# snuspl/parallax

Hardware: NVIDIA H100
Metric: lm1b_words_per_sec (higher is better)
Workload: dtype bf16

## Files before the change

### parallax_b200/ops/csrc/kernels/lstm_persistent.cu

```cuda
#include <cooperative_groups.h>
#include <mutex>

#include "wgmma.cuh"
#include "lstm_cell.cuh"

namespace cg = cooperative_groups;

namespace lstm_fwd {
using namespace tc;

constexpr int UNITS = 32;
constexpr int ROWS = 64;
constexpr int GN = 2 * UNITS;
constexpr int PN = 64;
constexpr int PK = 128;
constexpr int NTHREADS = 512;
constexpr int CELL_U = 4;
constexpr int GATE_LD = 4 * UNITS + 8;
constexpr int MAX_KB = 8;

struct Args {
  const __nv_bfloat16* xw;
  const __nv_bfloat16* Wh;
  const __nv_bfloat16* WP;
  __nv_bfloat16* act;
  float* c_all;
  __nv_bfloat16* m_all;
  __nv_bfloat16* h_all;
  float* ws;
  int T, S, P;
  float forget_bias;
};

__host__ __device__ constexpr int cmax(int a, int b) { return a > b ? a : b; }
__host__ __device__ constexpr int x_bytes(int P) {
  return cmax(cmax((P / BK) * ROWS * 128, (PK / BK) * BM * 128), ROWS * GATE_LD * 4);
}
__host__ __device__ constexpr int smem_bytes(int P) {
  return 2 * (P / BK) * GN * 128 + (PK / BK) * PN * 128 + x_bytes(P) + (MAX_KB + PK / BK) * 8 + 1024;
}
static_assert(smem_bytes(MAX_KB * BK) <= 232448, "P = 512 must fit one CTA's shared memory");

template <int N, typename Col>
__device__ __forceinline__ void load_transposed(uint8_t* dst, const __nv_bfloat16* src, size_t ld,
                                                int K, Col col) {
  const int nblk = (N / 8) * (K / 8);
  for (int b = threadIdx.x; b < nblk; b += blockDim.x) {
    const int n0 = (b % (N / 8)) * 8, k0 = (b / (N / 8)) * 8;
    uint4 v[8];
#pragma unroll
    for (int i = 0; i < 8; ++i)
      v[i] = __ldg(reinterpret_cast<const uint4*>(src + (size_t)(k0 + i) * ld + col(n0)));
    const uint32_t* w = reinterpret_cast<const uint32_t*>(v);
    uint8_t* blk = dst + (k0 / BK) * N * 128;
    const int c = (k0 % BK) / 8;
#pragma unroll
    for (int j = 0; j < 8; ++j) {
      const uint32_t sel = (j & 1) ? 0x7632u : 0x5410u;
      uint4 o;
      o.x = __byte_perm(w[0 * 4 + j / 2], w[1 * 4 + j / 2], sel);
      o.y = __byte_perm(w[2 * 4 + j / 2], w[3 * 4 + j / 2], sel);
      o.z = __byte_perm(w[4 * 4 + j / 2], w[5 * 4 + j / 2], sel);
      o.w = __byte_perm(w[6 * 4 + j / 2], w[7 * 4 + j / 2], sel);
      const int n = n0 + j;
      *reinterpret_cast<uint4*>(blk + n * 128 + ((c ^ (n & 7)) << 4)) = o;
    }
  }
}

__device__ __forceinline__ float2 bf16x2_to_float2(uint32_t w) {
  return make_float2(__uint_as_float(w << 16), __uint_as_float(w & 0xffff0000u));
}
__device__ __forceinline__ uint32_t float2_to_bf16x2(float a, float b) {
  __nv_bfloat162 h = __floats2bfloat162_rn(a, b);
  return *reinterpret_cast<uint32_t*>(&h);
}
__device__ __forceinline__ float round_bf16(float x) {
  return __bfloat162float(__float2bfloat16_rn(x));
}

__device__ __forceinline__ void product(float* acc, uint32_t a0, uint32_t a_stride, uint32_t b0,
                                        uint64_t* bar, int nkb, uint32_t parity) {
  for (int kb = 0; kb < nkb; ++kb) {
    mbar_wait(&bar[kb], parity);
    const uint64_t adesc = make_smem_desc(a0 + kb * a_stride);
    const uint64_t bdesc = make_smem_desc(b0 + kb * 64 * 128);
    wgmma_fence();
#pragma unroll
    for (int k = 0; k < BK / WG_K; ++k)
      wgmma_bf16<64>(acc, adesc + (uint64_t)(k * 2), bdesc + (uint64_t)(k * 2),
                     (kb | k) != 0 ? 1u : 0u);
    wgmma_commit();
  }
  wgmma_wait<0>();
}

__global__ void __launch_bounds__(NTHREADS, 1)
px_lstm_fwd_persistent_kernel(const __grid_constant__ CUtensorMap tmap_h,
                              const __grid_constant__ CUtensorMap tmap_m, Args a) {
  extern __shared__ __align__(1024) uint8_t smem_raw[];
  uint8_t* smem = reinterpret_cast<uint8_t*>(((uintptr_t)smem_raw + 1023) & ~(uintptr_t)1023);
  const int S = a.S, P = a.P, KB = P / BK;
  const size_t G4 = 4 * (size_t)S;
  uint8_t* sWh = smem;
  uint8_t* sWP = sWh + 2 * KB * GN * 128;
  uint8_t* sX = sWP + (PK / BK) * PN * 128;
  uint64_t* hbar = reinterpret_cast<uint64_t*>(sX + x_bytes(P));
  uint64_t* mbar = hbar + MAX_KB;

  const int row0 = (blockIdx.x & 1) * ROWS, u0 = (blockIdx.x >> 1) * UNITS;
  const int ntn = P / PN;
  const bool proj = (int)blockIdx.x < ntn * (S / PK);
  const int pn0 = (blockIdx.x % ntn) * PN, pk = blockIdx.x / ntn;

  if (threadIdx.x == 0) {
    asm volatile("prefetch.tensormap [%0];" ::"l"(&tmap_h) : "memory");
    asm volatile("prefetch.tensormap [%0];" ::"l"(&tmap_m) : "memory");
    for (int kb = 0; kb < KB; ++kb) mbar_init(&hbar[kb], 1);
    for (int kb = 0; kb < PK / BK; ++kb) mbar_init(&mbar[kb], 1);
    asm volatile("fence.mbarrier_init.release.cluster;" ::: "memory");
  }
  for (int w = 0; w < 2; ++w)
    load_transposed<GN>(sWh + w * KB * GN * 128, a.Wh, G4, P,
                        [=](int n) { return (n / 16) * S + u0 + 16 * w + n % 16; });
  if (proj)
    load_transposed<PN>(sWP, a.WP + (size_t)pk * PK * P, P, PK, [=](int n) { return pn0 + n; });
  asm volatile("fence.proxy.async.shared::cta;" ::: "memory");
  __syncthreads();

  const int wg = threadIdx.x >> 7, lane = threadIdx.x & 31, warp = (threadIdx.x >> 5) & 3;
  const int q2 = (lane & 3) * 2;
  const int r = warp * 16 + (lane >> 2);
  const int rb = wg * 64 + r;
  const int crow = threadIdx.x / (UNITS / CELL_U), cu = (threadIdx.x % (UNITS / CELL_U)) * CELL_U;
  const size_t cs_off = (size_t)(row0 + crow) * S + u0 + cu;
  const size_t cg_off = (size_t)(row0 + crow) * G4 + u0 + cu;
  float c[CELL_U];
  {
    const float4 v = *reinterpret_cast<const float4*>(a.c_all + cs_off);
    c[0] = v.x; c[1] = v.y; c[2] = v.z; c[3] = v.w;
  }
  float* sG = reinterpret_cast<float*>(sX);
  const uint32_t sX_u = smem_u32(sX), sWh_u = smem_u32(sWh) + (wg & 1) * KB * GN * 128;
  const uint32_t sWP_u = smem_u32(sWP);
  cg::grid_group grid = cg::this_grid();
  const int KS = S / PK;
  float acc[32];

  for (int t = 0; t < a.T; ++t) {
    const uint32_t parity = t & 1;
    if (threadIdx.x == 0) {
      asm volatile("fence.proxy.async.global;" ::: "memory");
      for (int kb = 0; kb < KB; ++kb) {
        mbar_expect_tx(&hbar[kb], ROWS * BK * 2);
        tma_load_2d(sX + kb * ROWS * 128, &tmap_h, &hbar[kb], kb * BK, t * BM + row0);
      }
    }
    uint2 xv[4];
    const __nv_bfloat16* xr = a.xw + (size_t)t * BM * G4 + cg_off;
#pragma unroll
    for (int g = 0; g < 4; ++g) xv[g] = __ldg(reinterpret_cast<const uint2*>(xr + (size_t)g * S));
    if (wg < 2) {
      product(acc, sX_u, ROWS * 128, sWh_u, hbar, KB, parity);
      consumer_sync();
#pragma unroll
      for (int h = 0; h < 2; ++h)
#pragma unroll
        for (int j = 0; j < GN / 8; ++j)
          *reinterpret_cast<float2*>(sG + (r + 8 * h) * GATE_LD + (j >> 1) * UNITS + wg * 16 +
                                     (j & 1) * 8 + q2) =
              make_float2(acc[j * 4 + 2 * h], acc[j * 4 + 2 * h + 1]);
    }
    __syncthreads();

    float av[4][CELL_U], mv[CELL_U];
#pragma unroll
    for (int g = 0; g < 4; ++g) {
      const float4 v = *reinterpret_cast<const float4*>(sG + crow * GATE_LD + g * UNITS + cu);
      const float2 lo = bf16x2_to_float2(xv[g].x), hi = bf16x2_to_float2(xv[g].y);
      av[g][0] = round_bf16(v.x + lo.x);
      av[g][1] = round_bf16(v.y + lo.y);
      av[g][2] = round_bf16(v.z + hi.x);
      av[g][3] = round_bf16(v.w + hi.y);
    }
    asm volatile("fence.proxy.async.shared::cta;" ::: "memory");
#pragma unroll
    for (int e = 0; e < CELL_U; ++e) {
      float ae[4];
      c[e] = lstm_cell_fwd_elem(av[0][e], av[1][e], av[2][e], av[3][e], c[e], a.forget_bias, ae,
                                &mv[e]);
#pragma unroll
      for (int g = 0; g < 4; ++g) av[g][e] = ae[g];
    }
    __nv_bfloat16* act = a.act + (size_t)t * BM * G4 + cg_off;
#pragma unroll
    for (int g = 0; g < 4; ++g)
      *reinterpret_cast<uint2*>(act + (size_t)g * S) =
          make_uint2(float2_to_bf16x2(av[g][0], av[g][1]), float2_to_bf16x2(av[g][2], av[g][3]));
    *reinterpret_cast<float4*>(a.c_all + (size_t)(t + 1) * BM * S + cs_off) =
        make_float4(c[0], c[1], c[2], c[3]);
    *reinterpret_cast<uint2*>(a.m_all + (size_t)t * BM * S + cs_off) =
        make_uint2(float2_to_bf16x2(mv[0], mv[1]), float2_to_bf16x2(mv[2], mv[3]));
    grid.sync();

    if (proj && wg < 2) {
      if (threadIdx.x == 0) {
        asm volatile("fence.proxy.async.global;" ::: "memory");
        for (int kb = 0; kb < PK / BK; ++kb) {
          mbar_expect_tx(&mbar[kb], BM * BK * 2);
          tma_load_2d(sX + kb * BM * 128, &tmap_m, &mbar[kb], pk * PK + kb * BK, t * BM);
        }
      }
      product(acc, sX_u + wg * 64 * 128, BM * 128, sWP_u, mbar, PK / BK, parity);
      float* slot = a.ws + (size_t)pk * BM * P;
#pragma unroll
      for (int h = 0; h < 2; ++h)
#pragma unroll
        for (int j = 0; j < PN / 8; ++j)
          *reinterpret_cast<float2*>(slot + (size_t)(rb + 8 * h) * P + pn0 + j * 8 + q2) =
              make_float2(acc[j * 4 + 2 * h], acc[j * 4 + 2 * h + 1]);
    }
    grid.sync();

    __nv_bfloat16* hn = a.h_all + (size_t)(t + 1) * BM * P;
    const int npairs = BM * P / 2;
    for (int i = blockIdx.x * blockDim.x + threadIdx.x; i < npairs; i += gridDim.x * blockDim.x) {
      float2 s = __ldcg(reinterpret_cast<const float2*>(a.ws) + i);
#pragma unroll 8
      for (int k = 1; k < KS; ++k) {
        const float2 v = __ldcg(reinterpret_cast<const float2*>(a.ws + (size_t)k * BM * P) + i);
        s.x += v.x;
        s.y += v.y;
      }
      reinterpret_cast<uint32_t*>(hn)[i] = float2_to_bf16x2(s.x, s.y);
    }
    if (t + 1 < a.T) grid.sync();
  }
}

}

extern "C" {

int px_lstm_fwd_persistent_grid(int B, int S, int P) {
  using namespace lstm_fwd;
  if (B != BM || S <= 0 || S % PK || P <= 0 || P % PN || P > MAX_KB * BK) return 0;
  static std::mutex mu;
  static int cap[16][MAX_KB + 1];
  int dev = 0;
  if (cudaGetDevice(&dev) != cudaSuccess || dev < 0 || dev >= 16) return 0;
  std::lock_guard<std::mutex> lock(mu);
  int& n = cap[dev][P / PN];
  if (n == 0) {
    int coop = 0, sms = 0, per_sm = 0;
    cudaDeviceGetAttribute(&coop, cudaDevAttrCooperativeLaunch, dev);
    cudaDeviceGetAttribute(&sms, cudaDevAttrMultiProcessorCount, dev);
    const int smem = smem_bytes(P);
    if (cudaFuncSetAttribute(px_lstm_fwd_persistent_kernel,
                             cudaFuncAttributeMaxDynamicSharedMemorySize,
                             smem_bytes(MAX_KB * BK)) != cudaSuccess ||
        cudaOccupancyMaxActiveBlocksPerMultiprocessor(&per_sm, px_lstm_fwd_persistent_kernel,
                                                      NTHREADS, smem) != cudaSuccess)
      per_sm = 0;
    n = (coop && per_sm > 0) ? per_sm * sms : -1;
    cudaGetLastError();
  }
  const int grid = 2 * (S / UNITS);
  return n >= grid ? grid : 0;
}

int px_lstm_fwd_persistent(const void* xw, const void* Wh, const void* WP, void* act, float* c_all,
                           void* m_all, void* h_all, float* ws, int T, int B, int S, int P,
                           float forget_bias, cudaStream_t stream) {
  using namespace lstm_fwd;
  const int grid = px_lstm_fwd_persistent_grid(B, S, P);
  if (grid <= 0 || T < 1) return -1;
  for (const void* q : {xw, Wh, WP, (const void*)act, (const void*)c_all, (const void*)m_all,
                        (const void*)h_all, (const void*)ws})
    if ((uintptr_t)q % 16) return -1;
  CUtensorMap th, tm;
  int rc = make_tmap(&th, h_all, (uint64_t)(T + 1) * B, P, ROWS);
  if (rc) return rc;
  rc = make_tmap(&tm, m_all, (uint64_t)T * B, S, BM);
  if (rc) return rc;
  Args a;
  a.xw = (const __nv_bfloat16*)xw; a.Wh = (const __nv_bfloat16*)Wh;
  a.WP = (const __nv_bfloat16*)WP; a.act = (__nv_bfloat16*)act; a.c_all = c_all;
  a.m_all = (__nv_bfloat16*)m_all; a.h_all = (__nv_bfloat16*)h_all; a.ws = ws;
  a.T = T; a.S = S; a.P = P; a.forget_bias = forget_bias;
  cudaLaunchConfig_t cfg = {};
  cfg.gridDim = dim3(grid);
  cfg.blockDim = dim3(NTHREADS);
  cfg.dynamicSmemBytes = smem_bytes(P);
  cfg.stream = stream;
  cudaLaunchAttribute at[1];
  at[0].id = cudaLaunchAttributeCooperative;
  at[0].val.cooperative = 1;
  cfg.attrs = at;
  cfg.numAttrs = 1;
  const cudaError_t e = cudaLaunchKernelEx(&cfg, px_lstm_fwd_persistent_kernel, th, tm, a);
  return e == cudaSuccess ? (int)cudaGetLastError() : (int)e;
}

}
```

### parallax_b200/ops/fused.py

```python
import ctypes

import torch

from . import lib as _lib, check as _check, register_signatures

_vp, _i, _f = ctypes.c_void_p, ctypes.c_int, ctypes.c_float
register_signatures({
    "px_lstm_cell_fwd": (_i, [_vp, _vp, _vp, _vp, _vp, _i, _i, _f, _i, _vp]),
    "px_lstm_cell_bwd": (_i, [_vp, _vp, _vp, _vp, _vp, _vp, _i, _i, _i, _vp]),
    "px_lstm_dm_cell_bwd": (_i, [_vp] * 7 + [_i, _i, _i, _i, _vp]),
    "px_lstm_fwd_persistent_grid": (_i, [_i, _i, _i]),
    "px_lstm_fwd_persistent": (_i, [_vp] * 8 + [_i, _i, _i, _i, _f, _vp]),
    "px_sampled_softmax": (_i, [_vp, _vp, _vp, _vp, _vp, _vp, _vp, _vp, _i, _i, _i, _vp]),
    "px_sampled_softmax_dot": (_i, [_vp, _vp, _vp, _i, _vp, _vp, _vp, _vp, _vp, _vp, _i, _i, _i,
                                    _vp]),
    "px_ssm_bwd": (_i, [_vp, _vp, _vp, _vp, _i, _vp, _vp, _f, _vp, _vp, _vp, _i, _vp, _i, _i, _i,
                        _vp]),
})
_DT = {torch.float32: 0, torch.bfloat16: 1}


def _p(t):
    return _vp(t.data_ptr())


def _stream():
    return _vp(torch.cuda.current_stream().cuda_stream)


def _count(n=1):
    from ..parallel import nvops
    nvops.launches["n"] += n


def _acc(t):
    return t if t.dtype == torch.float64 else t.float()


BWD_BN = 16


def _fused_bwd_ok(dt, Bsz, S, P, W_P):
    return (dt == torch.bfloat16 and Bsz % 128 == 0 and S % BWD_BN == 0 and P % 64 == 0 and
            W_P.is_contiguous() and W_P.data_ptr() % 16 == 0)


_persistent_grid = {}


def _fwd_persistent_ok(dt, Bsz, S, P, Wh, W_P):
    if not (dt == torch.bfloat16 and Wh.is_contiguous() and W_P.is_contiguous() and
            Wh.data_ptr() % 16 == 0 and W_P.data_ptr() % 16 == 0):
        return False
    key = (torch.cuda.current_device(), Bsz, S, P)
    if key not in _persistent_grid:
        _persistent_grid[key] = _lib().px_lstm_fwd_persistent_grid(Bsz, S, P)
    return _persistent_grid[key] > 0


def lstm_layer_reference(x, Wx, Wh, bias, W_P, c0, h0, forget_bias=1.0):
    T, Bsz, E = x.shape
    S = W_P.shape[0]
    xw = torch.addmm(bias, x.reshape(T * Bsz, E), Wx).view(T, Bsz, 4 * S)
    c, h, outs = _acc(c0), h0, []
    for t in range(T):
        gates = _acc(torch.addmm(xw[t], h, Wh))
        i, j, f, o = gates.split(S, dim=1)
        c = torch.sigmoid(f + forget_bias) * c + torch.sigmoid(i) * torch.tanh(j)
        m = (torch.sigmoid(o) * torch.tanh(c)).to(x.dtype)
        h = m @ W_P
        outs.append(h)
    return torch.stack(outs), c, h


class _LSTMLayerFn(torch.autograd.Function):

    @staticmethod
    def forward(ctx, x, W, Wh, bias, W_P, c0, h0, forget_bias):
        L = _lib()
        T, Bsz, E = x.shape
        S, P = W_P.shape
        dt = x.dtype
        dev = x.device
        x = x.contiguous()
        stacked = Wh is None
        ctx.stacked = stacked
        ctx.param_refs = (W, bias, W_P)
        if stacked:
            Wx, Wh = W.detach()[:E], W.detach()[E:]
        else:
            Wx = W
        if any(ctx.needs_input_grad) and not _fused_bwd_ok(dt, Bsz, S, P, W_P):
            from . import sinks
            cur = torch.cuda.current_stream(dev)
            ws = sinks.side_stream(dev)
            ws.wait_stream(cur)
            with torch.cuda.stream(ws):
                ctx.WPT = W_P.detach().t().contiguous()
                ctx.WPT_ev = torch.cuda.Event()
                ctx.WPT_ev.record(ws)
            ctx.WPT.record_stream(cur)
        xw = torch.addmm(bias, x.view(T * Bsz, E), Wx).view(T, Bsz, 4 * S)
        act = torch.empty(T, Bsz, 4 * S, dtype=dt, device=dev)
        c_all = torch.empty(T + 1, Bsz, S, dtype=torch.float32, device=dev)
        m_all = torch.empty(T, Bsz, S, dtype=dt, device=dev)
        h_all = torch.empty(T + 1, Bsz, P, dtype=dt, device=dev)
        c_all[0].copy_(c0)
        h_all[0].copy_(h0)
        st = _stream()
        if _fwd_persistent_ok(dt, Bsz, S, P, Wh, W_P):
            ws = torch.empty(S // 128, Bsz, P, dtype=torch.float32, device=dev)
            _check(L.px_lstm_fwd_persistent(_p(xw), _p(Wh), _p(W_P), _p(act), _p(c_all),
                                            _p(m_all), _p(h_all), _p(ws), T, Bsz, S, P,
                                            float(forget_bias), st), "lstm_fwd_persistent")
            _count(1)
        else:
            for t in range(T):
                gpre = xw[t].addmm_(h_all[t], Wh)
                _check(L.px_lstm_cell_fwd(_p(gpre), _p(c_all[t]), _p(act[t]),
                                          _p(c_all[t + 1]), _p(m_all[t]), Bsz, S,
                                          float(forget_bias), _DT[dt], st), "lstm_cell_fwd")
                torch.mm(m_all[t], W_P, out=h_all[t + 1])
            _count(T)
        ctx.save_for_backward(x, Wx, Wh, W_P, act, c_all, m_all, h_all)
        ctx.dims = (T, Bsz, E, S, P)
        return h_all[1:], c_all[T].clone(), h_all[T].clone()

    @staticmethod
    def backward(ctx, dH, dcT, dhT):
        from . import sinks
        L = _lib()
        x, Wx, Wh, W_P, act, c_all, m_all, h_all = ctx.saved_tensors
        T, Bsz, E, S, P = ctx.dims
        stacked = ctx.stacked
        W_ref, bias_ref, WP_ref = ctx.param_refs
        dt, dev = x.dtype, x.device
        dH = dH.contiguous()
        dgates = torch.empty(T, Bsz, 4 * S, dtype=dt, device=dev)
        dh_tot = torch.empty(T, Bsz, P, dtype=dt, device=dev)
        dc = torch.zeros(Bsz, S, dtype=torch.float32, device=dev) if dcT is None \
            else dcT.float().clone()
        dh_rec = None if dhT is None else dhT.to(dt)
        fused = _fused_bwd_ok(dt, Bsz, S, P, W_P)
        dm = None if fused else torch.empty(Bsz, S, dtype=dt, device=dev)
        cur = torch.cuda.current_stream(dev)
        if not fused:
            cur.wait_event(ctx.WPT_ev)
            WPT = ctx.WPT
        from . import gemm as _gemm
        use_tc = (dt == torch.bfloat16 and Bsz % 128 == 0 and P % 64 == 0 and
                  (4 * S) % 1024 == 0 and Wh.is_contiguous())
        WhT = None if use_tc else Wh.t().contiguous()
        st = _stream()

        def sink_of(ref, shape):
            s_ = sinks.get(ref)
            if s_ is not None and s_.dtype == dt and tuple(s_.shape) == tuple(shape):
                return s_, True
            return torch.empty(shape, dtype=dt, device=dev), False
        if stacked:
            dW, w_sunk = sink_of(W_ref, (E + P, 4 * S))
            dWx_o, dWh_o = dW[:E], dW[E:]
        else:
            dWx_o, w_sunk = sink_of(W_ref, (E, 4 * S))
            dWh_o = torch.empty(P, 4 * S, dtype=dt, device=dev)
        dbias_o, b_sunk = sink_of(bias_ref, (4 * S,))
        dWP_o, p_sunk = sink_of(WP_ref, (S, P))
        ws = sinks.side_stream(dev)
        ws2 = sinks.side_stream(dev, 1)
        if dh_rec is None:
            dh_tot[T - 1].copy_(dH[T - 1])
        else:
            torch.add(dH[T - 1], dh_rec, out=dh_tot[T - 1])
        for t in range(T - 1, -1, -1):
            if fused:
                _check(L.px_lstm_dm_cell_bwd(_p(dh_tot[t]), _p(W_P), _p(dc), _p(act[t]),
                                             _p(c_all[t]), _p(c_all[t + 1]), _p(dgates[t]), Bsz,
                                             S, P, BWD_BN, st), "lstm_dm_cell_bwd")
            else:
                torch.mm(dh_tot[t], WPT, out=dm)
                _check(L.px_lstm_cell_bwd(_p(dm), _p(dc), _p(act[t]), _p(c_all[t]),
                                          _p(c_all[t + 1]), _p(dgates[t]), Bsz, S, _DT[dt], st),
                       "lstm_cell_bwd")
            if t > 0:
                if use_tc:
                    _gemm.gemm_tn(dgates[t], Wh, addend=dH[t - 1], splits=8, bn=64,
                                  out=dh_tot[t - 1])
                else:
                    torch.addmm(dH[t - 1], dgates[t], WhT, out=dh_tot[t - 1])
            else:
                dh_rec = _gemm.gemm_tn(dgates[0], Wh, splits=8, bn=64) if use_tc \
                    else torch.mm(dgates[0], WhT)
        _count(T)
        dg2 = dgates.view(T * Bsz, 4 * S)
        ws2.wait_stream(cur)
        with torch.cuda.stream(ws2):
            torch.sum(dg2, 0, out=dbias_o)
        ev_b = torch.cuda.Event()
        ev_b.record(ws2)
        dgates.record_stream(ws2)
        dbias_o.record_stream(ws2)
        dx = (dg2 @ Wx.t()).view(T, Bsz, E)
        ws.wait_stream(cur)
        with torch.cuda.stream(ws):
            torch.mm(h_all[:T].reshape(-1, P).t(), dg2, out=dWh_o)
            torch.mm(x.reshape(-1, E).t(), dg2, out=dWx_o)
            torch.mm(m_all.reshape(-1, S).t(), dh_tot.view(-1, P), out=dWP_o)
        ev = torch.cuda.Event()
        ev.record(ws)
        for t_ in (dgates, dh_tot, x, h_all, m_all, dWh_o, dWx_o, dbias_o, dWP_o):
            t_.record_stream(ws)
        outs, plain = [], False
        for ref, o, sunk, e_ in ((W_ref, dW if stacked else dWx_o, w_sunk, ev),
                                 (bias_ref, dbias_o, b_sunk, ev_b), (WP_ref, dWP_o, p_sunk, ev)):
            if sunk:
                sinks.deliver(ref, e_)
                outs.append(None)
            else:
                outs.append(o)
                plain = True
        if plain or not stacked:
            cur.wait_event(ev)
            cur.wait_event(ev_b)
        dW_out, dbias, dW_P = outs
        return dx, dW_out, None if stacked else dWh_o, dbias, dW_P, dc, dh_rec, None


def lstm_layer(x, Wx, Wh, bias, W_P, c0, h0, forget_bias=1.0):
    if x.is_cuda and x.dtype in _DT:
        return _LSTMLayerFn.apply(x, Wx, Wh, bias, W_P, c0, h0, forget_bias)
    return lstm_layer_reference(x, Wx, Wh, bias, W_P, c0, h0, forget_bias)


def lstm_layer_stacked(x, W, bias, W_P, c0, h0, forget_bias=1.0):
    E = x.shape[-1]
    if x.is_cuda and x.dtype in _DT:
        return _LSTMLayerFn.apply(x, W, None, bias, W_P, c0, h0, forget_bias)
    return lstm_layer_reference(x, W[:E], W[E:], bias, W_P, c0, h0, forget_bias)


def sampled_softmax_reference(inputs, true_w, samp_w, true_b, samp_b, logq_true,
                              logq_samp, targets, sampled):
    true_logits = _acc((inputs * true_w).sum(-1)) + _acc(true_b) - logq_true
    samp_logits = _acc(inputs @ samp_w.t()) + (_acc(samp_b) - logq_samp)
    hits = targets.unsqueeze(1) == sampled.unsqueeze(0)
    samp_logits = samp_logits.masked_fill(hits, float("-inf"))
    lse = torch.logsumexp(torch.cat([true_logits.unsqueeze(1), samp_logits], 1), 1)
    return lse - true_logits


class _SampledSoftmaxFn(torch.autograd.Function):
    @staticmethod
    def forward(ctx, inputs, true_w, samp_w, true_b, samp_b, logq_true, logq_samp,
                targets, sampled):
        L = _lib()
        N, S = inputs.shape[0], samp_w.shape[0]
        dt = inputs.dtype
        logits = inputs @ samp_w.t()
        true_dot = (inputs.float() * true_w.float()).sum(-1)
        adj_t = (true_b.float() - logq_true).contiguous()
        adj_s = (samp_b.float() - logq_samp).contiguous()
        loss = torch.empty(N, dtype=torch.float32, device=inputs.device)
        dtrue = torch.empty(N, dtype=torch.float32, device=inputs.device)
        tg = targets.to(torch.int64).contiguous()
        sm = sampled.to(torch.int64).contiguous()
        _check(L.px_sampled_softmax(_p(logits), _p(true_dot), _p(adj_t), _p(adj_s), _p(tg),
                                    _p(sm), _p(loss), _p(dtrue), N, S, _DT[dt], _stream()),
               "sampled_softmax")
        _count(1)
        ctx.save_for_backward(inputs, true_w, samp_w, logits, dtrue)
        return loss

    @staticmethod
    def backward(ctx, g):
        inputs, true_w, samp_w, probs, dtrue = ctx.saved_tensors
        dt = inputs.dtype
        g = g.float()
        gt = (g * dtrue).unsqueeze(1)
        d_inputs = ((probs @ samp_w).float() * g.unsqueeze(1) +
                    gt * true_w.float()).to(dt)
        gi = (inputs.float() * g.unsqueeze(1)).to(dt)
        d_samp_w = probs.t() @ gi
        d_true_w = (gt * inputs.float()).to(dt)
        d_samp_b = (probs.float().t() @ g) if probs.dtype == torch.float32 else \
            torch.mm(probs.t(), g.to(dt).unsqueeze(1), out_dtype=torch.float32).squeeze(1)
        d_true_b = gt.squeeze(1)
        return d_inputs, d_true_w, d_samp_w, d_true_b, d_samp_b, None, None, None, None


def sampled_softmax_loss(inputs, true_w, samp_w, true_b, samp_b, logq_true, logq_samp,
                         targets, sampled):
    if inputs.is_cuda and inputs.dtype in _DT and samp_w.shape[0] <= 256 * 64:
        return _SampledSoftmaxFn.apply(inputs, true_w.to(inputs.dtype),
                                       samp_w.to(inputs.dtype), true_b, samp_b,
                                       logq_true, logq_samp, targets, sampled)
    return sampled_softmax_reference(inputs, true_w, samp_w, true_b, samp_b, logq_true,
                                     logq_samp, targets, sampled)


def _head_forward(inputs, w_all, adj, targets, sampled):
    N, S = inputs.shape[0], w_all.shape[0] - inputs.shape[0]
    P = inputs.shape[1]
    logits = inputs @ w_all[N:].t()
    if inputs.is_cuda:
        loss = torch.empty(N, dtype=torch.float32, device=inputs.device)
        dtrue = torch.empty(N, dtype=torch.float32, device=inputs.device)
        _check(_lib().px_sampled_softmax_dot(
            _p(logits), _p(inputs), _p(w_all), P, _p(adj), _vp(adj.data_ptr() + 4 * N),
            _p(targets), _p(sampled), _p(loss), _p(dtrue), N, S, _DT[inputs.dtype], _stream()),
            "sampled_softmax_dot")
        _count(1)
        return logits, loss, dtrue
    tl = (inputs.float() * w_all[:N].float()).sum(-1) + adj[:N]
    a = logits.float() + adj[N:]
    a = a.masked_fill(targets.unsqueeze(1) == sampled.unsqueeze(0), float("-inf"))
    mx = torch.maximum(a.max(1).values, tl)
    e, et = torch.exp(a - mx.unsqueeze(1)), torch.exp(tl - mx)
    denom = e.sum(1) + et
    return (e / denom.unsqueeze(1)).to(inputs.dtype), mx + torch.log(denom) - tl, et / denom - 1.0


def _head_backward(G, inputs, w_all, g, row_w, dtrue, gi, d_w_all, db, grow):
    N, P = inputs.shape
    if inputs.is_cuda:
        _check(_lib().px_ssm_bwd(
            _p(G), _p(inputs), _p(w_all), _p(g), 0 if g.numel() == 1 else 1,
            _p(row_w) if row_w is not None else None, _p(dtrue), 1.0 / N, _p(gi), _p(d_w_all),
            _p(db), 1 if db.dtype == torch.bfloat16 else 0, _p(grow), N, P, _DT[inputs.dtype],
            _stream()), "ssm_bwd")
        _count(1)
        return
    gr = g.reshape(-1).float() * (1.0 / N)
    gr = gr.expand(N) if gr.numel() == 1 else gr
    if row_w is not None:
        gr = gr * row_w
    gt = gr * dtrue
    x, wt = inputs.float(), w_all[:N].float()
    G.copy_(G.float() * gr.unsqueeze(1) + gt.unsqueeze(1) * wt)
    gi.copy_(x * gr.unsqueeze(1))
    d_w_all[:N].copy_(x * gt.unsqueeze(1))
    db[:N].copy_(gt)
    grow.copy_(gr)


class _SampledSoftmaxHeadFn(torch.autograd.Function):

    @staticmethod
    def forward(ctx, inputs, w_all, b_all, adj, targets, sampled, row_w):
        probs, loss, dtrue = _head_forward(inputs, w_all, adj, targets, sampled)
        ctx.save_for_backward(inputs, w_all, probs, dtrue, row_w)
        ctx.b_meta = (tuple(b_all.shape), b_all.dtype)
        if row_w is not None:
            loss = loss * row_w
        return loss.mean()

    @staticmethod
    def backward(ctx, g):
        inputs, w_all, probs, dtrue, row_w = ctx.saved_tensors
        N, P = inputs.shape
        S = w_all.shape[0] - N
        dt, dev = inputs.dtype, inputs.device
        b_shape, b_dt = ctx.b_meta
        g = g.float().contiguous()
        G = probs @ w_all[N:]
        d_w_all = torch.empty(N + S, P, dtype=dt, device=dev)
        db = torch.empty(N + S, dtype=b_dt if b_dt in _DT else torch.float32, device=dev)
        gi = torch.empty(N, P, dtype=dt, device=dev)
        grow = torch.empty(N, dtype=dt, device=dev)
        _head_backward(G, inputs, w_all, g, row_w, dtrue, gi, d_w_all, db, grow)
        torch.mm(probs.t(), gi, out=d_w_all[N:])
        if db.dtype == dt:
            torch.mm(probs.t(), grow.view(N, 1), out=db[N:].view(S, 1))
        elif dt == torch.bfloat16 and db.dtype == torch.float32:
            db[N:].copy_(torch.mm(probs.t(), grow.view(N, 1), out_dtype=torch.float32).view(S))
        else:
            db[N:].copy_((probs.t() @ grow.view(N, 1)).view(S))
        db = db.view(b_shape)
        if db.dtype != b_dt:
            db = db.to(b_dt)
        return G, d_w_all, db, None, None, None, None


def sampled_softmax_head(inputs, w_all, b_all, logq, targets, sampled, row_w=None, adj=None):
    N, P = inputs.shape
    S = w_all.shape[0] - N
    dt = inputs.dtype
    vec = 4 if dt == torch.float32 else 8
    fused = (inputs.is_cuda and dt in _DT and w_all.dtype == dt and
             0 < S <= 256 * 64 and P % vec == 0 and b_all.numel() == N + S)
    if fused:
        inputs = inputs.contiguous()
        w_all = w_all.contiguous()
        fused = inputs.data_ptr() % 16 == 0 and w_all.data_ptr() % 16 == 0
    if not fused:
        b = b_all.reshape(-1)
        loss = sampled_softmax_loss(inputs, w_all[:N], w_all[N:], b[:N], b[N:], logq[:N],
                                    logq[N:], targets, sampled)
        if row_w is not None:
            loss = loss * row_w.to(loss.dtype)
        return loss.mean()
    if adj is None:
        adj = b_all.detach().reshape(-1).float() - logq
    adj = adj.float().contiguous()
    tg = targets.to(torch.int64).contiguous()
    sm = sampled.to(torch.int64).contiguous()
    rw = None if row_w is None else row_w.detach().float().contiguous()
    return _SampledSoftmaxHeadFn.apply(inputs, w_all, b_all, adj, tg, sm, rw)
```

Before: 2.010 million.

## Add persistent cooperative kernel for LSTM backward recurrence

Result: faster. 2.141 million (median of 6 runs) (+6.5%).

```diff
diff --git a/parallax_b200/ops/csrc/kernels/lstm_persistent.cu b/parallax_b200/ops/csrc/kernels/lstm_persistent.cu
--- a/parallax_b200/ops/csrc/kernels/lstm_persistent.cu
+++ b/parallax_b200/ops/csrc/kernels/lstm_persistent.cu
@@ -79,17 +79,19 @@
   return __bfloat162float(__float2bfloat16_rn(x));
 }
 
+template <int N>
 __device__ __forceinline__ void product(float* acc, uint32_t a0, uint32_t a_stride, uint32_t b0,
-                                        uint64_t* bar, int nkb, uint32_t parity) {
+                                        uint32_t b_stride, uint64_t* bar, int nkb,
+                                        uint32_t parity) {
   for (int kb = 0; kb < nkb; ++kb) {
     mbar_wait(&bar[kb], parity);
     const uint64_t adesc = make_smem_desc(a0 + kb * a_stride);
-    const uint64_t bdesc = make_smem_desc(b0 + kb * 64 * 128);
+    const uint64_t bdesc = make_smem_desc(b0 + kb * b_stride);
     wgmma_fence();
 #pragma unroll
     for (int k = 0; k < BK / WG_K; ++k)
-      wgmma_bf16<64>(acc, adesc + (uint64_t)(k * 2), bdesc + (uint64_t)(k * 2),
-                     (kb | k) != 0 ? 1u : 0u);
+      wgmma_bf16<N>(acc, adesc + (uint64_t)(k * 2), bdesc + (uint64_t)(k * 2),
+                    (kb | k) != 0 ? 1u : 0u);
     wgmma_commit();
   }
   wgmma_wait<0>();
@@ -161,7 +163,7 @@
 #pragma unroll
     for (int g = 0; g < 4; ++g) xv[g] = __ldg(reinterpret_cast<const uint2*>(xr + (size_t)g * S));
     if (wg < 2) {
-      product(acc, sX_u, ROWS * 128, sWh_u, hbar, KB, parity);
+      product<GN>(acc, sX_u, ROWS * 128, sWh_u, GN * 128, hbar, KB, parity);
       consumer_sync();
 #pragma unroll
       for (int h = 0; h < 2; ++h)
@@ -211,7 +213,7 @@
           tma_load_2d(sX + kb * BM * 128, &tmap_m, &mbar[kb], pk * PK + kb * BK, t * BM);
         }
       }
-      product(acc, sX_u + wg * 64 * 128, BM * 128, sWP_u, mbar, PK / BK, parity);
+      product<PN>(acc, sX_u + wg * 64 * 128, BM * 128, sWP_u, PN * 128, mbar, PK / BK, parity);
       float* slot = a.ws + (size_t)pk * BM * P;
 #pragma unroll
       for (int h = 0; h < 2; ++h)
@@ -238,35 +240,272 @@
   }
 }
 
-}
-
-extern "C" {
-
-int px_lstm_fwd_persistent_grid(int B, int S, int P) {
-  using namespace lstm_fwd;
-  if (B != BM || S <= 0 || S % PK || P <= 0 || P % PN || P > MAX_KB * BK) return 0;
+template <auto Kernel, int (*Smem)(int)>
+int persistent_grid(int grid, int P) {
   static std::mutex mu;
   static int cap[16][MAX_KB + 1];
   int dev = 0;
   if (cudaGetDevice(&dev) != cudaSuccess || dev < 0 || dev >= 16) return 0;
   std::lock_guard<std::mutex> lock(mu);
-  int& n = cap[dev][P / PN];
+  int& n = cap[dev][P / BK];
   if (n == 0) {
     int coop = 0, sms = 0, per_sm = 0;
     cudaDeviceGetAttribute(&coop, cudaDevAttrCooperativeLaunch, dev);
     cudaDeviceGetAttribute(&sms, cudaDevAttrMultiProcessorCount, dev);
-    const int smem = smem_bytes(P);
-    if (cudaFuncSetAttribute(px_lstm_fwd_persistent_kernel,
-                             cudaFuncAttributeMaxDynamicSharedMemorySize,
-                             smem_bytes(MAX_KB * BK)) != cudaSuccess ||
-        cudaOccupancyMaxActiveBlocksPerMultiprocessor(&per_sm, px_lstm_fwd_persistent_kernel,
-                                                      NTHREADS, smem) != cudaSuccess)
+    if (cudaFuncSetAttribute(Kernel, cudaFuncAttributeMaxDynamicSharedMemorySize,
+                             Smem(MAX_KB * BK)) != cudaSuccess ||
+        cudaOccupancyMaxActiveBlocksPerMultiprocessor(&per_sm, Kernel, NTHREADS, Smem(P)) !=
+            cudaSuccess)
       per_sm = 0;
     n = (coop && per_sm > 0) ? per_sm * sms : -1;
     cudaGetLastError();
   }
-  const int grid = 2 * (S / UNITS);
   return n >= grid ? grid : 0;
+}
+
+template <typename... KArgs, typename... Args>
+int launch_cooperative(void (*kernel)(KArgs...), int grid, int smem, cudaStream_t stream,
+                       Args... args) {
+  cudaLaunchConfig_t cfg = {};
+  cfg.gridDim = dim3(grid);
+  cfg.blockDim = dim3(NTHREADS);
+  cfg.dynamicSmemBytes = smem;
+  cfg.stream = stream;
+  cudaLaunchAttribute at[1];
+  at[0].id = cudaLaunchAttributeCooperative;
+  at[0].val.cooperative = 1;
+  cfg.attrs = at;
+  cfg.numAttrs = 1;
+  const cudaError_t e = cudaLaunchKernelEx(&cfg, kernel, args...);
+  return e == cudaSuccess ? (int)cudaGetLastError() : (int)e;
+}
+
+}
+
+namespace lstm_bwd {
+using namespace lstm_fwd;
+
+constexpr int WN = 64;
+constexpr int WK = 512;
+constexpr int DM_LD = UNITS + 8;
+
+struct Args {
+  const __nv_bfloat16* dH;
+  const __nv_bfloat16* act;
+  const float* c_all;
+  float* dc;
+  __nv_bfloat16* dgates;
+  __nv_bfloat16* dh_tot;
+  __nv_bfloat16* dh_rec;
+  float* ws;
+  int T, S, P;
+};
+
+__host__ __device__ constexpr int wp_bytes(int P) { return (P / BK) * UNITS * 128; }
+__host__ __device__ constexpr int x_bytes(int P) {
+  return cmax(cmax((P / BK) * ROWS * 128, (WK / BK) * BM * 128), ROWS * DM_LD * 4);
+}
+__host__ __device__ constexpr int smem_bytes(int P) {
+  return (WK / BK) * WN * 128 + wp_bytes(P) + x_bytes(P) + (MAX_KB + WK / BK + 1) * 8 + 1024;
+}
+static_assert(smem_bytes(MAX_KB * BK) <= 232448, "P = 512 must fit one CTA's shared memory");
+static_assert(WN / 2 >= UNITS / 2, "the accumulator holds phase 1's tile too");
+
+__global__ void __launch_bounds__(NTHREADS, 1)
+px_lstm_bwd_persistent_kernel(const __grid_constant__ CUtensorMap tmap_dh,
+                              const __grid_constant__ CUtensorMap tmap_wp,
+                              const __grid_constant__ CUtensorMap tmap_dg,
+                              const __grid_constant__ CUtensorMap tmap_wh, Args a) {
+  extern __shared__ __align__(1024) uint8_t smem_raw[];
+  uint8_t* smem = reinterpret_cast<uint8_t*>(((uintptr_t)smem_raw + 1023) & ~(uintptr_t)1023);
+  const int S = a.S, P = a.P, KB = P / BK;
+  const size_t G4 = 4 * (size_t)S;
+  uint8_t* sWh = smem;
+  uint8_t* sWP = sWh + (WK / BK) * WN * 128;
+  uint8_t* sX = sWP + wp_bytes(P);
+  uint64_t* hbar = reinterpret_cast<uint64_t*>(sX + x_bytes(P));
+  uint64_t* gbar = hbar + MAX_KB;
+  uint64_t* wbar = gbar + WK / BK;
+
+  const int row0 = (blockIdx.x & 1) * ROWS, u0 = (blockIdx.x >> 1) * UNITS;
+  const int ntn = P / WN, NS = (int)(G4 / WK);
+  const bool item = (int)blockIdx.x < ntn * NS;
+  const int n0 = (blockIdx.x % ntn) * WN, ks = blockIdx.x / ntn;
+
+  if (threadIdx.x == 0) {
+    asm volatile("prefetch.tensormap [%0];" ::"l"(&tmap_dh) : "memory");
+    asm volatile("prefetch.tensormap [%0];" ::"l"(&tmap_wp) : "memory");
+    asm volatile("prefetch.tensormap [%0];" ::"l"(&tmap_dg) : "memory");
+    asm volatile("prefetch.tensormap [%0];" ::"l"(&tmap_wh) : "memory");
+    for (int kb = 0; kb < KB; ++kb) mbar_init(&hbar[kb], 1);
+    for (int kb = 0; kb < WK / BK; ++kb) mbar_init(&gbar[kb], 1);
+    mbar_init(wbar, 1);
+    asm volatile("fence.mbarrier_init.release.cluster;" ::: "memory");
+    mbar_expect_tx(wbar, wp_bytes(P) + (item ? (WK / BK) * WN * 128 : 0));
+    for (int kb = 0; kb < KB; ++kb)
+      tma_load_2d(sWP + kb * UNITS * 128, &tmap_wp, wbar, kb * BK, u0);
+    if (item)
+      for (int kb = 0; kb < WK / BK; ++kb)
+        tma_load_2d(sWh + kb * WN * 128, &tmap_wh, wbar, ks * WK + kb * BK, n0);
+  }
+  __syncthreads();
+
+  const int wg = threadIdx.x >> 7, lane = threadIdx.x & 31, warp = (threadIdx.x >> 5) & 3;
+  const int q2 = (lane & 3) * 2;
+  const int r = warp * 16 + (lane >> 2);
+  const int crow = threadIdx.x / (UNITS / CELL_U), cu = (threadIdx.x % (UNITS / CELL_U)) * CELL_U;
+  const size_t cs_off = (size_t)(row0 + crow) * S + u0 + cu;
+  const size_t cg_off = (size_t)(row0 + crow) * G4 + u0 + cu;
+  float dc[CELL_U];
+  {
+    const float4 v = *reinterpret_cast<const float4*>(a.dc + cs_off);
+    dc[0] = v.x; dc[1] = v.y; dc[2] = v.z; dc[3] = v.w;
+  }
+  float* sD = reinterpret_cast<float*>(sX);
+  const uint32_t sX_u0 = smem_u32(sX), sWP_u0 = smem_u32(sWP), sWh_u0 = smem_u32(sWh);
+  cg::grid_group grid = cg::this_grid();
+  float acc[WN / 4];
+  mbar_wait(wbar, 0);
+
+  for (int t = a.T - 1; t >= 0; --t) {
+    const uint32_t parity = (a.T - 1 - t) & 1;
+    uint32_t sX_u = sX_u0, sWP_u = sWP_u0, sWh_u = sWh_u0;
+    asm volatile("" : "+r"(sX_u), "+r"(sWP_u), "+r"(sWh_u));
+    if (threadIdx.x == 0) {
+      asm volatile("fence.proxy.async.global;" ::: "memory");
+      for (int kb = 0; kb < KB; ++kb) {
+        mbar_expect_tx(&hbar[kb], ROWS * BK * 2);
+        tma_load_2d(sX + kb * ROWS * 128, &tmap_dh, &hbar[kb], kb * BK, t * BM + row0);
+      }
+    }
+    uint2 av[4];
+    const __nv_bfloat16* ar = a.act + (size_t)t * BM * G4 + cg_off;
+#pragma unroll
+    for (int g = 0; g < 4; ++g) av[g] = __ldg(reinterpret_cast<const uint2*>(ar + (size_t)g * S));
+    const float4 cp = __ldg(reinterpret_cast<const float4*>(a.c_all + (size_t)t * BM * S + cs_off));
+    const float4 cn =
+        __ldg(reinterpret_cast<const float4*>(a.c_all + (size_t)(t + 1) * BM * S + cs_off));
+    if (wg < 2) {
+      product<UNITS / 2>(acc, sX_u, ROWS * 128, sWP_u + wg * (UNITS / 2) * 128, UNITS * 128, hbar,
+                         KB, parity);
+      consumer_sync();
+#pragma unroll
+      for (int h = 0; h < 2; ++h)
+#pragma unroll
+        for (int j = 0; j < UNITS / 16; ++j)
+          *reinterpret_cast<float2*>(sD + (r + 8 * h) * DM_LD + wg * 16 + j * 8 + q2) =
+              make_float2(round_bf16(acc[j * 4 + 2 * h]), round_bf16(acc[j * 4 + 2 * h + 1]));
+    }
+    __syncthreads();
+    const float4 dm = *reinterpret_cast<const float4*>(sD + crow * DM_LD + cu);
+    asm volatile("fence.proxy.async.shared::cta;" ::: "memory");
+    float ag[4][CELL_U];
+#pragma unroll
+    for (int g = 0; g < 4; ++g) {
+      const float2 lo = bf16x2_to_float2(av[g].x), hi = bf16x2_to_float2(av[g].y);
+      ag[g][0] = lo.x; ag[g][1] = lo.y; ag[g][2] = hi.x; ag[g][3] = hi.y;
+    }
+    const float dmv[CELL_U] = {dm.x, dm.y, dm.z, dm.w}, cpv[CELL_U] = {cp.x, cp.y, cp.z, cp.w},
+                cnv[CELL_U] = {cn.x, cn.y, cn.z, cn.w};
+#pragma unroll
+    for (int e = 0; e < CELL_U; ++e) {
+      const float ae[4] = {ag[0][e], ag[1][e], ag[2][e], ag[3][e]};
+      float dge[4];
+      dc[e] = lstm_cell_bwd_elem(ae, cpv[e], cnv[e], dmv[e], dc[e], dge);
+#pragma unroll
+      for (int g = 0; g < 4; ++g) ag[g][e] = dge[g];
+    }
+    __nv_bfloat16* dg = a.dgates + (size_t)t * BM * G4 + cg_off;
+#pragma unroll
+    for (int g = 0; g < 4; ++g)
+      *reinterpret_cast<uint2*>(dg + (size_t)g * S) =
+          make_uint2(float2_to_bf16x2(ag[g][0], ag[g][1]), float2_to_bf16x2(ag[g][2], ag[g][3]));
+    grid.sync();
+
+    if (item) {
+      if (threadIdx.x == 0) {
+        asm volatile("fence.proxy.async.global;" ::: "memory");
+        for (int kb = 0; kb < WK / BK; ++kb) {
+          mbar_expect_tx(&gbar[kb], BM * BK * 2);
+          tma_load_2d(sX + kb * BM * 128, &tmap_dg, &gbar[kb], ks * WK + kb * BK, t * BM);
+        }
+      }
+      product<WN / 2>(acc, sX_u + (wg & 1) * 64 * 128, BM * 128,
+                      sWh_u + (wg >> 1) * (WN / 2) * 128, WN * 128, gbar, WK / BK, parity);
+      float* slot = a.ws + (size_t)ks * BM * P;
+      const int rb = (wg & 1) * 64 + r, cb = n0 + (wg >> 1) * (WN / 2);
+#pragma unroll
+      for (int h = 0; h < 2; ++h)
+#pragma unroll
+        for (int j = 0; j < WN / 16; ++j)
+          *reinterpret_cast<float2*>(slot + (size_t)(rb + 8 * h) * P + cb + j * 8 + q2) =
+              make_float2(acc[j * 4 + 2 * h], acc[j * 4 + 2 * h + 1]);
+    }
+    grid.sync();
+
+    __nv_bfloat16* out = t > 0 ? a.dh_tot + (size_t)(t - 1) * BM * P : a.dh_rec;
+    const uint32_t* add =
+        reinterpret_cast<const uint32_t*>(a.dH + (size_t)(t > 0 ? t - 1 : 0) * BM * P);
+    const int npairs = BM * P / 2;
+    for (int i = blockIdx.x * blockDim.x + threadIdx.x; i < npairs; i += gridDim.x * blockDim.x) {
+      float2 s = __ldcg(reinterpret_cast<const float2*>(a.ws) + i);
+#pragma unroll 8
+      for (int k = 1; k < NS; ++k) {
+        const float2 v = __ldcg(reinterpret_cast<const float2*>(a.ws + (size_t)k * BM * P) + i);
+        s.x += v.x;
+        s.y += v.y;
+      }
+      if (t > 0) {
+        const float2 d = bf16x2_to_float2(__ldg(add + i));
+        s.x += d.x;
+        s.y += d.y;
+      }
+      reinterpret_cast<uint32_t*>(out)[i] = float2_to_bf16x2(s.x, s.y);
+    }
+    if (t > 0) grid.sync();
+  }
+  *reinterpret_cast<float4*>(a.dc + cs_off) = make_float4(dc[0], dc[1], dc[2], dc[3]);
+}
+
+}
+
+extern "C" {
+
+int px_lstm_fwd_persistent_grid(int B, int S, int P) {
+  using namespace lstm_fwd;
+  if (B != BM || S <= 0 || S % PK || P <= 0 || P % PN || P > MAX_KB * BK) return 0;
+  return persistent_grid<px_lstm_fwd_persistent_kernel, smem_bytes>(2 * (S / UNITS), P);
+}
+
+int px_lstm_bwd_persistent_grid(int B, int S, int P) {
+  using namespace lstm_fwd;
+  if (B != BM || S <= 0 || S % 128 || P <= 0 || P % lstm_bwd::WN || P > MAX_KB * BK) return 0;
+  return persistent_grid<lstm_bwd::px_lstm_bwd_persistent_kernel, lstm_bwd::smem_bytes>(
+      2 * (S / UNITS), P);
+}
+
+int px_lstm_bwd_persistent(const void* dH, const void* act, const float* c_all, const void* Wh,
+                           const void* WP, float* dc, void* dgates, void* dh_tot, void* dh_rec,
+                           float* ws, int T, int B, int S, int P, cudaStream_t stream) {
+  using namespace lstm_fwd;
+  const int grid = px_lstm_bwd_persistent_grid(B, S, P);
+  if (grid <= 0 || T < 1) return -1;
+  for (const void* q : {dH, act, (const void*)c_all, Wh, WP, (const void*)dc, (const void*)dgates,
+                        (const void*)dh_tot, (const void*)dh_rec, (const void*)ws})
+    if ((uintptr_t)q % 16) return -1;
+  CUtensorMap tdh, twp, tdg, twh;
+  int rc = make_tmap(&tdh, dh_tot, (uint64_t)T * B, P, ROWS);
+  if (!rc) rc = make_tmap(&twp, WP, S, P, UNITS);
+  if (!rc) rc = make_tmap(&tdg, dgates, (uint64_t)T * B, 4 * (uint64_t)S, BM);
+  if (!rc) rc = make_tmap(&twh, Wh, P, 4 * (uint64_t)S, lstm_bwd::WN);
+  if (rc) return rc;
+  lstm_bwd::Args a;
+  a.dH = (const __nv_bfloat16*)dH; a.act = (const __nv_bfloat16*)act; a.c_all = c_all;
+  a.dc = dc; a.dgates = (__nv_bfloat16*)dgates; a.dh_tot = (__nv_bfloat16*)dh_tot;
+  a.dh_rec = (__nv_bfloat16*)dh_rec; a.ws = ws;
+  a.T = T; a.S = S; a.P = P;
+  return launch_cooperative(lstm_bwd::px_lstm_bwd_persistent_kernel, grid,
+                            lstm_bwd::smem_bytes(P), stream, tdh, twp, tdg, twh, a);
 }
 
 int px_lstm_fwd_persistent(const void* xw, const void* Wh, const void* WP, void* act, float* c_all,
@@ -288,18 +527,7 @@
   a.WP = (const __nv_bfloat16*)WP; a.act = (__nv_bfloat16*)act; a.c_all = c_all;
   a.m_all = (__nv_bfloat16*)m_all; a.h_all = (__nv_bfloat16*)h_all; a.ws = ws;
   a.T = T; a.S = S; a.P = P; a.forget_bias = forget_bias;
-  cudaLaunchConfig_t cfg = {};
-  cfg.gridDim = dim3(grid);
-  cfg.blockDim = dim3(NTHREADS);
-  cfg.dynamicSmemBytes = smem_bytes(P);
-  cfg.stream = stream;
-  cudaLaunchAttribute at[1];
-  at[0].id = cudaLaunchAttributeCooperative;
-  at[0].val.cooperative = 1;
-  cfg.attrs = at;
-  cfg.numAttrs = 1;
-  const cudaError_t e = cudaLaunchKernelEx(&cfg, px_lstm_fwd_persistent_kernel, th, tm, a);
-  return e == cudaSuccess ? (int)cudaGetLastError() : (int)e;
-}
-
-}
+  return launch_cooperative(px_lstm_fwd_persistent_kernel, grid, smem_bytes(P), stream, th, tm, a);
+}
+
+}
diff --git a/parallax_b200/ops/fused.py b/parallax_b200/ops/fused.py
--- a/parallax_b200/ops/fused.py
+++ b/parallax_b200/ops/fused.py
@@ -11,6 +11,8 @@
     "px_lstm_dm_cell_bwd": (_i, [_vp] * 7 + [_i, _i, _i, _i, _vp]),
     "px_lstm_fwd_persistent_grid": (_i, [_i, _i, _i]),
     "px_lstm_fwd_persistent": (_i, [_vp] * 8 + [_i, _i, _i, _i, _f, _vp]),
+    "px_lstm_bwd_persistent_grid": (_i, [_i, _i, _i]),
+    "px_lstm_bwd_persistent": (_i, [_vp] * 10 + [_i, _i, _i, _i, _vp]),
     "px_sampled_softmax": (_i, [_vp, _vp, _vp, _vp, _vp, _vp, _vp, _vp, _i, _i, _i, _vp]),
     "px_sampled_softmax_dot": (_i, [_vp, _vp, _vp, _i, _vp, _vp, _vp, _vp, _vp, _vp, _i, _i, _i,
                                     _vp]),
@@ -48,14 +50,22 @@
 _persistent_grid = {}
 
 
-def _fwd_persistent_ok(dt, Bsz, S, P, Wh, W_P):
+def _persistent_ok(entry, dt, Bsz, S, P, Wh, W_P):
     if not (dt == torch.bfloat16 and Wh.is_contiguous() and W_P.is_contiguous() and
             Wh.data_ptr() % 16 == 0 and W_P.data_ptr() % 16 == 0):
         return False
-    key = (torch.cuda.current_device(), Bsz, S, P)
+    key = (entry, torch.cuda.current_device(), Bsz, S, P)
     if key not in _persistent_grid:
-        _persistent_grid[key] = _lib().px_lstm_fwd_persistent_grid(Bsz, S, P)
+        _persistent_grid[key] = getattr(_lib(), entry)(Bsz, S, P)
     return _persistent_grid[key] > 0
+
+
+def _fwd_persistent_ok(dt, Bsz, S, P, Wh, W_P):
+    return _persistent_ok("px_lstm_fwd_persistent_grid", dt, Bsz, S, P, Wh, W_P)
+
+
+def _bwd_persistent_ok(dt, Bsz, S, P, Wh, W_P):
+    return _persistent_ok("px_lstm_bwd_persistent_grid", dt, Bsz, S, P, Wh, W_P)
 
 
 def lstm_layer_reference(x, Wx, Wh, bias, W_P, c0, h0, forget_bias=1.0):
@@ -172,26 +182,34 @@
             dh_tot[T - 1].copy_(dH[T - 1])
         else:
             torch.add(dH[T - 1], dh_rec, out=dh_tot[T - 1])
-        for t in range(T - 1, -1, -1):
-            if fused:
-                _check(L.px_lstm_dm_cell_bwd(_p(dh_tot[t]), _p(W_P), _p(dc), _p(act[t]),
-                                             _p(c_all[t]), _p(c_all[t + 1]), _p(dgates[t]), Bsz,
-                                             S, P, BWD_BN, st), "lstm_dm_cell_bwd")
-            else:
-                torch.mm(dh_tot[t], WPT, out=dm)
-                _check(L.px_lstm_cell_bwd(_p(dm), _p(dc), _p(act[t]), _p(c_all[t]),
-                                          _p(c_all[t + 1]), _p(dgates[t]), Bsz, S, _DT[dt], st),
-                       "lstm_cell_bwd")
-            if t > 0:
-                if use_tc:
-                    _gemm.gemm_tn(dgates[t], Wh, addend=dH[t - 1], splits=8, bn=64,
-                                  out=dh_tot[t - 1])
+        if _bwd_persistent_ok(dt, Bsz, S, P, Wh, W_P) and dH.data_ptr() % 16 == 0:
+            dh_rec = torch.empty(Bsz, P, dtype=dt, device=dev)
+            ws_ = torch.empty(4 * S // 512, Bsz, P, dtype=torch.float32, device=dev)
+            _check(L.px_lstm_bwd_persistent(_p(dH), _p(act), _p(c_all), _p(Wh), _p(W_P), _p(dc),
+                                            _p(dgates), _p(dh_tot), _p(dh_rec), _p(ws_), T, Bsz,
+                                            S, P, st), "lstm_bwd_persistent")
+            _count(1)
+        else:
+            for t in range(T - 1, -1, -1):
+                if fused:
+                    _check(L.px_lstm_dm_cell_bwd(_p(dh_tot[t]), _p(W_P), _p(dc), _p(act[t]),
+                                                 _p(c_all[t]), _p(c_all[t + 1]), _p(dgates[t]),
+                                                 Bsz, S, P, BWD_BN, st), "lstm_dm_cell_bwd")
                 else:
-                    torch.addmm(dH[t - 1], dgates[t], WhT, out=dh_tot[t - 1])
-            else:
-                dh_rec = _gemm.gemm_tn(dgates[0], Wh, splits=8, bn=64) if use_tc \
-                    else torch.mm(dgates[0], WhT)
-        _count(T)
+                    torch.mm(dh_tot[t], WPT, out=dm)
+                    _check(L.px_lstm_cell_bwd(_p(dm), _p(dc), _p(act[t]), _p(c_all[t]),
+                                              _p(c_all[t + 1]), _p(dgates[t]), Bsz, S, _DT[dt],
+                                              st), "lstm_cell_bwd")
+                if t > 0:
+                    if use_tc:
+                        _gemm.gemm_tn(dgates[t], Wh, addend=dH[t - 1], splits=8, bn=64,
+                                      out=dh_tot[t - 1])
+                    else:
+                        torch.addmm(dH[t - 1], dgates[t], WhT, out=dh_tot[t - 1])
+                else:
+                    dh_rec = _gemm.gemm_tn(dgates[0], Wh, splits=8, bn=64) if use_tc \
+                        else torch.mm(dgates[0], WhT)
+            _count(T)
         dg2 = dgates.view(T * Bsz, 4 * S)
         ws2.wait_stream(cur)
         with torch.cuda.stream(ws2):
```
